# nerficg-project/nerficg

Hardware: AMD Instinct MI355X
Metric: Mrays/s (INGP lego) (higher is better)
Workload: dtype f16 (tables, weights, activations) / f32 (accumulate, march, composite); 1 GPU; ingp_lego: 800x800 image render per rank per step (640000 rays), solid-sphere occupancy r<0.35, random-init hash grid (T=2^19, L=16, F=2) + 64-wide MLPs, seed 0, 100 seeded orbit poses; parallelism=rays x1 (weak)

## Files before the change

### include/nerficg_hip.h

```cpp
#ifndef NERFICG_HIP_H
#define NERFICG_HIP_H

#include <stdint.h>

#ifdef __cplusplus
extern "C" {
#endif

typedef void* nrc_stream_t;

enum {
    NRC_OK = 0,
    NRC_ERR_INVALID = -1,
    NRC_ERR_LAUNCH = -2,
    NRC_ERR_UNSUPPORTED = -3
};

#define NRC_ABI_VERSION 22
int nrc_abi_version(void);
const char* nrc_build_info(void);
const char* nrc_last_error(void);


int nrc_ray_aabb_intersect(const float* rays_o, const float* rays_d, const float* centers, const float* half_sizes,
// ... 269 lines not shown
                             void* view, nrc_stream_t stream);
int nrc_ngp_set_encoder_ypair_view(const void* view);
int nrc_ngp_set_encoder_ypair_levels(int32_t levels);
int nrc_ngp_encode_samples(const float* ts, const int32_t* row_tile, const float* ray_od, int64_t first_row, int64_t n_rows, const float* xyz_min3,
                           const float* xyz_size3, const void* table_f16, int32_t n_levels, int32_t log2_hashmap_size,
                           int32_t base_resolution, float per_level_scale, void* features_f16, const int32_t* arena_tile_off,
                           int32_t arena_rows, nrc_stream_t stream);
int nrc_ngp_mlp_samples(const float* ts, const int32_t* row_tile, const float* ray_od, int64_t first_row, int64_t n_rows, int64_t n_ray_tiles,
                        const void* features_f16, const void* density_weights_f16, const void* color_weights_f16,
                        void* packed_f16, void* ray_sh_workspace, const int32_t* arena_tile_off, int32_t arena_rows, nrc_stream_t stream);
int nrc_ngp_composite_image(const void* packed_f16, const float* ts, const int32_t* ray_cnt, const int32_t* tile_off,
                            int32_t width, int32_t height, int64_t tile_begin, int64_t n_tiles, int32_t cascades,
                            float exp_step_factor, int32_t grid_size, int32_t max_samples, float T_threshold,
                            const float* bg3, float* rgb, float* alpha, float* depth, int64_t row_capacity, int32_t arena_rows,
                            nrc_stream_t stream);
int64_t nrc_ngp_render_frame_ws_bytes(int64_t n_rows, int64_t n_ray_tiles, int32_t max_samples, int64_t row_budget);
int nrc_ngp_render_frame(const float* ts_arena, int32_t* row_tile, const float* ray_od, int64_t n_rows, int64_t n_ray_tiles,
                         const float* xyz_min3, const float* xyz_size3, const void* density_weights_f16, const void* color_weights_f16,
                         const void* table_f16, int32_t n_levels, int32_t log2_hashmap_size, int32_t base_resolution, float per_level_scale,
                         const int32_t* ray_cnt, const int32_t* tile_off, int32_t width, int32_t height, int64_t tile_begin, int32_t cascades,
                         float exp_step_factor, int32_t grid_size, int32_t max_samples, float T_threshold, const float* bg3_host, float* rgb,
                         float* alpha, float* depth, int64_t row_budget, void* workspace, nrc_stream_t stream);

int nrc_ssim_forward(const float* img1, const float* img2, int64_t planes, int32_t H, int32_t W, float C1, float C2, float* ssim_map,
                     float* dm_dmu1, float* dm_dsigma1_sq, float* dm_dsigma12, nrc_stream_t stream);
int nrc_ssim_backward(const float* img1, const float* img2, int64_t planes, int32_t H, int32_t W, const float* dL_dmap,
                      const float* dm_dmu1, const float* dm_dsigma1_sq, const float* dm_dsigma12, float* dL_dimg1,
                      nrc_stream_t stream);
int64_t nrc_photometric_loss_ws_floats(int64_t planes, int32_t H, int32_t W);
int nrc_photometric_loss_forward(const float* image, const float* target, int64_t planes, int32_t H, int32_t W, float C1, float C2,
// ... 229 lines not shown
```

### nerficg_amd/csrc/ngp_net.hip

```cpp
#include "ngp_net.h"
#include "ngp_image_step.h"

namespace {

enum { ENC_GRID = 0, ENC_SH_ID = 1, ENC_FEAT = 2, ENC_DIR_H = 3, ENC_GRID_F2 = 4, ENC_GRID_F4 = 5 };
enum { ACT_NONE = 0, ACT_SIGMOID = 1 };

__device__ __forceinline__ void encode_grid(float px, float py, float pz, int hh, __amdgpu_buffer_rsrc_t table, const GridCfg& g, h8 (&B)[2]) {
#pragma unroll
    for (int s = 0; s < 2; s++) {
#pragma unroll
        for (int q = 0; q < 4; q++) {
            const int l0 = 8 * s + q, l1 = 8 * s + 4 + q;
            const float scale = hh ? g.scale[l1] : g.scale[l0];
            const uint32_t res = hh ? g.res[l1] : g.res[l0];
            const uint32_t size = hh ? g.size[l1] : g.size[l0];
            const uint32_t off = hh ? g.offset[l1] : g.offset[l0];
            const bool hashed = hh ? g.hashed[l1] : g.hashed[l0];
            Corner8 c;
            grid_corners(px, py, pz, scale, res, size, off, hashed, c);
            float f0, f1;
            grid_level_features(table, c, f0, f1);
            B[s][2 * q] = (_Float16)f0;
            B[s][2 * q + 1] = (_Float16)f1;
// ... 226 lines not shown
            px = __fdiv_rn(px, in.sz[0]); py = __fdiv_rn(py, in.sz[1]); pz = __fdiv_rn(pz, in.sz[2]);
        }
        return 1;
    }
}
template <int SRC>
__device__ __forceinline__ void fetch_dir(const QueryIn& in, int64_t i, float& dx, float& dy, float& dz) {
    if constexpr (SRC == SRC_ARRAYS) {
        dx = in.dirs[3 * i]; dy = in.dirs[3 * i + 1]; dz = in.dirs[3 * i + 2];
    } else {
        const float* od = in.ray_od + (int64_t)tile_of(in.row_tile[i >> 6]) * 384 + (i & 63);
        dx = od[192]; dy = od[256]; dz = od[320];
    }
}

template <int SRC>
__global__ void __launch_bounds__(256) k_grid_encode(QueryIn in, int64_t base, int64_t n, const __half2* __restrict__ table, GridCfg g,
                                                         uint4* __restrict__ feat, int narrow_levels, int lvl_range, int lane_shape = 0, int xcd_run = 0,
                                                         BlockView bv = BlockView{}, VertexView vv = VertexView{}, YPairView yv = YPairView{}) {
    int64_t bid = blockIdx.x;
    if constexpr (SRC == SRC_TILED) {
        int64_t first = 0, span = gridDim.x;
        if (xcd_run > 0) {
            const int64_t run = 8 * (int64_t)xcd_run;
            first = bid / run * run;
            span = first + run <= (int64_t)gridDim.x ? run : (int64_t)gridDim.x - first;
        }
        const int64_t g8 = span >> 3, r = bid - first;
        if (r < 8 * g8) bid = first + (r & 7) * g8 + (r >> 3);
    }
    int64_t j = bid * 256 + threadIdx.x;
    bool remapped = false;
    if constexpr (SRC == SRC_TILED) {
        if (in.n_rows_dev) {
// ... 5 lines not shown
            base = r0 * 64;
            n = (r1 - r0) * 64 < n ? (r1 - r0) * 64 : n;
        }
    }
    if constexpr (SRC == SRC_TILED) {
        if (lane_shape != 0) {
            const int lu = (lane_shape >> 4) & 7, lv = lane_shape & 7, ls = 6 - lu - lv;
            const int64_t g1024 = j & ~(int64_t)1023;
            const int w = (int)((j >> 6) & 15), l = (int)(j & 63);
            const int iu = l & ((1 << lu) - 1), iv = (l >> lu) & ((1 << lv) - 1), is = l >> (lu + lv);
            const int gu = w & ((NRC_TILE_W >> lu) - 1), gv = (w >> (NRC_TILE_W_LOG2 - lu)) & ((NRC_TILE_H >> lv) - 1), gs = w >> (6 - lu - lv);
            j = g1024 + ((int64_t)((gs << ls) + is) << 6) + NRC_TILE_W * ((gv << lv) + iv) + (gu << lu) + iu;
            remapped = true;
        }
    }
    if (j >= n || j < 0) return;
    float px, py, pz;
    if (blockIdx.y != 0) in.x01_out = nullptr;
    const int state = remapped ? fetch_pos<SRC, false>(in, base + j, px, py, pz) : fetch_pos<SRC>(in, base + j, px, py, pz);
    if (state < 0) return;
    const bool live = state > 0;
    const __amdgpu_buffer_rsrc_t trs = make_table_rsrc(table, g.total_entries * 4u);
    const __amdgpu_buffer_rsrc_t vrs = make_table_rsrc(bv.ptr, bv.bytes);
    const __amdgpu_buffer_rsrc_t xrs = make_table_rsrc(vv.ptr, vv.bytes);
    const __amdgpu_buffer_rsrc_t yrs = make_table_rsrc(yv.ptr, yv.bytes);
    uint4* out = feat + ((j >> 5) * 4) * 32 + (j & 31);
    const int rot = (int)((j >> 5) & 3);
    const int lvl_lo = lvl_range & 0xff, lvl_hi = (lvl_range >> 8) & 0xff;
    const int grp_begin = gridDim.y == 4 ? (int)blockIdx.y : 0, grp_end = gridDim.y == 4 ? grp_begin + 1 : 4;
#pragma unroll 1
    for (int grp = grp_begin; grp < grp_end; grp++) {
        uint32_t v[4] = {0u, 0u, 0u, 0u};
        if (live) {
#pragma unroll
            for (int q = 0; q < 4; q++) {
                const int level = 4 * grp + q;
                if (level < lvl_lo || level >= lvl_hi) continue;
                Corner8 c;
                float f0, f1;
                if (SRC == SRC_TILED && level < bv.levels) {
                    uint32_t gx, gy, gz;
                    grid_cell(px, py, pz, g.scale[level], gx, gy, gz, c.w);
                    grid_level_features_block(vrs, bv.first[level], gx, gy, gz, g.res[level], c.w, f0, f1);
                } else if (SRC == SRC_TILED && level >= yv.begin && level < yv.begin + yv.levels) {
// ... 5 lines not shown
                    grid_cell(px, py, pz, g.scale[level], gx, gy, gz, c.w);
                    grid_level_features_vertex(xrs, vv.first[level - vv.begin], gx, gy, gz, g.res[level], vv.R[level - vv.begin], c.w, f0, f1);
                } else if (g.hashed[level]) {
                    grid_corners_u<true>(px, py, pz, g.scale[level], g.res[level], g.size[level], g.offset[level], c);
                    grid_level_features_hashed(trs, c, f0, f1);
                } else {
                    grid_corners_u<false>(px, py, pz, g.scale[level], g.res[level], g.size[level], g.offset[level], c);
                    if (level < narrow_levels) grid_level_features_narrow(trs, c, f0, f1);
                    else grid_level_features(trs, c, f0, f1);
                }
                const __half2 h = __floats2half2_rn(f0, f1);
                v[q] = *reinterpret_cast<const uint32_t*>(&h);
                asm volatile("" : "+v"(v[q]));
            }
        }
        out[((grp + rot) & 3) * 32] = make_uint4(v[0], v[1], v[2], v[3]);
    }
}

__global__ void __launch_bounds__(256) k_grid_encode_pairs(QueryIn in, int64_t n, const __half2* __restrict__ table, GridCfg g, uint2* __restrict__ feat,
                                                           int narrow_levels, const int32_t* __restrict__ m_live = nullptr) {
    const int pair = (int)(blockIdx.x & 7u);
    const int64_t j = (int64_t)(blockIdx.x >> 3) * 256 + threadIdx.x;
    if (m_live) n = min(n, ((int64_t)max(*m_live, 0) + 31) / 32 * 32);
    if (j >= n) return;
    float px, py, pz;
    if (pair != 0) in.x01_out = nullptr;
    fetch_pos<SRC_ARRAYS>(in, j, px, py, pz);
    const __amdgpu_buffer_rsrc_t trs = make_table_rsrc(table, g.total_entries * 4u);
    uint32_t* out32 = reinterpret_cast<uint32_t*>(feat);
    const int rot = (int)((j >> 5) & 3);
// ... 70 lines not shown
    const float* od = ray_od + tile * 384 + lane;
    h8 lo, hi;
    sh4_fragments(od[192], od[256], od[320], lo, hi);
    ray_sh[(tile * 2) * 64 + lane] = lo;
    ray_sh[(tile * 2 + 1) * 64 + lane] = hi;
}

__device__ __forceinline__ float fast_sigmoid(float x) { return __builtin_amdgcn_rcpf(1.f + __expf(-x)); }

__device__ __forceinline__ h8 mlp_frag_relu(const f16v& acc, int g) { return acc_to_frag_relu(acc, g); }
__device__ __forceinline__ h8 mlp_frag(const f16v& acc, int g) { return acc_to_frag(acc, g); }
__device__ __forceinline__ f16v mlp_mfma(const h8& a, const h8& b, const f16v& c) { return NRC_MFMA(a, b, c); }
#ifndef NRC_MLP_WAVES
#define NRC_MLP_WAVES 2
#endif
enum { MLP_F_D0 = 0, MLP_F_DO = 4, MLP_F_C0 = 8, MLP_F_C1 = 12, MLP_F_CO = 20, MLP_N_FRAG = 24 };
__device__ __forceinline__ void mlp_stage_weights(h8 (*wlds)[64], const __half* __restrict__ Wd, const __half* __restrict__ Wc) {
    const int lane = threadIdx.x & 63, r = lane & 31, hh = lane >> 5;
    for (int f = threadIdx.x >> 6; f < MLP_N_FRAG; f += 4) {
        h8 v;
        if (f < MLP_F_DO) v = load_w_frag<false>(Wd, 32, 64, (f - MLP_F_D0) >> 1, (f - MLP_F_D0) & 1, r, hh);
        else if (f < MLP_F_C0) v = load_w_head_frag(Wd + 64 * 32, 64, 16, (f - MLP_F_DO) & 1, lane);
        else if (f < MLP_F_C1) {
            const int mt = (f - MLP_F_C0) >> 1, s = (f - MLP_F_C0) & 1;
            v = load_w_frag<false>(Wc, 32, 64, mt, s, r, hh);
        } else if (f < MLP_F_CO) v = load_w_frag<true>(Wc + 64 * 32, 64, 64, (f - MLP_F_C1) >> 2, (f - MLP_F_C1) & 3, r, hh);
        else v = load_w_head_frag(Wc + 64 * 32 + 64 * 64, 64, 16, (f - MLP_F_CO) & 1, lane);
        wlds[f][lane] = v;
    }
}
template <int NT, bool PRE>
__device__ __forceinline__ void mlp_chain_from(const h8 (*wlds)[64], const h8 (&B)[NT][2], const h8 (*X0), const f16v (*P)[2],
                                               _Float16 (&h0)[NT], _Float16 (&rgbh)[NT][3]) {
    const int lane = threadIdx.x & 63;
#define D0(mt, s) wlds[MLP_F_D0 + 2 * (mt) + (s)][lane]
#define DO(s) wlds[MLP_F_DO + (s)][lane]
#define C0(mt, s) wlds[MLP_F_C0 + 2 * (mt) + (s)][lane]
#define C1(mt, s) wlds[MLP_F_C1 + 4 * (mt) + (s)][lane]
#define CO(s) wlds[MLP_F_CO + (s)][lane]
    h8 X[NT][2], H[NT][4];
    f16v acc[NT][2];
    h8 HB[NT][2][2];
    f4v o[NT][2];
#pragma unroll
    for (int u = 0; u < NT; u++) {
        if constexpr (!PRE) X[u][0] = X0[u];
        acc[u][0] = zero16(); acc[u][1] = zero16();
        o[u][0] = f4v{0.f, 0.f, 0.f, 0.f}; o[u][1] = o[u][0];
    }
#pragma unroll
    for (int mt = 0; mt < 2; mt++)
#pragma unroll
        for (int s = 0; s < 2; s++) {
            const h8 w = D0(mt, s);
#pragma unroll
            for (int u = 0; u < NT; u++) acc[u][mt] = mlp_mfma(w, B[u][s], acc[u][mt]);
        }
#pragma unroll
    for (int u = 0; u < NT; u++) {
#pragma unroll
        for (int mt = 0; mt < 2; mt++)
#pragma unroll
            for (int gq = 0; gq < 2; gq++) H[u][2 * mt + gq] = mlp_frag_relu(acc[u][mt], gq);
        head_split(H[u], HB[u]);
    }
#pragma unroll
    for (int s = 0; s < 2; s++) {
        const h8 w = DO(s);
#pragma unroll
        for (int u = 0; u < NT; u++)
#pragma unroll
            for (int nb = 0; nb < 2; nb++) o[u][nb] = NRC_MFMA16(w, HB[u][nb][s], o[u][nb]);
    }
#pragma unroll
    for (int u = 0; u < NT; u++) {
        X[u][1] = head_join(o[u][0], o[u][1]);
        h0[u] = X[u][1][0];
        if constexpr (!PRE) { acc[u][0] = zero16(); acc[u][1] = zero16(); }
    }
#pragma unroll
    for (int mt = 0; mt < 2; mt++)
#pragma unroll
        for (int s = PRE ? 1 : 0; s < 2; s++) {
            const h8 w = C0(mt, s);
#pragma unroll
            for (int u = 0; u < NT; u++) {
                if constexpr (PRE) acc[u][mt] = mlp_mfma(w, X[u][1], P[u][mt]);
                else acc[u][mt] = mlp_mfma(w, X[u][s], acc[u][mt]);
            }
        }
#pragma unroll
    for (int u = 0; u < NT; u++) {
#pragma unroll
        for (int mt = 0; mt < 2; mt++)
#pragma unroll
            for (int gq = 0; gq < 2; gq++) H[u][2 * mt + gq] = mlp_frag_relu(acc[u][mt], gq);
        acc[u][0] = zero16(); acc[u][1] = zero16();
    }
#pragma unroll
    for (int mt = 0; mt < 2; mt++)
#pragma unroll
        for (int s = 0; s < 4; s++) {
            const h8 w = C1(mt, s);
// ... 12 lines not shown
#pragma unroll
    for (int s = 0; s < 2; s++) {
        const h8 w = CO(s);
#pragma unroll
        for (int u = 0; u < NT; u++)
#pragma unroll
            for (int nb = 0; nb < 2; nb++) o[u][nb] = NRC_MFMA16(w, HB[u][nb][s], o[u][nb]);
    }
#pragma unroll
    for (int u = 0; u < NT; u++) {
        float rgb[3];
        head_join_rgb(o[u][0], o[u][1], rgb);
#pragma unroll
        for (int c = 0; c < 3; c++) rgbh[u][c] = (_Float16)fast_sigmoid(rgb[c]);
    }
#undef D0
#undef DO
#undef C1
#undef CO
}
template <int NT>
__device__ __forceinline__ void mlp_chain(const h8 (*wlds)[64], const h8 (&B)[NT][2], const h8 (&X0)[NT], _Float16 (&h0)[NT], _Float16 (&rgbh)[NT][3]) {
    mlp_chain_from<NT, false>(wlds, B, X0, nullptr, h0, rgbh);
}
template <int NT>
__device__ __forceinline__ void mlp_chain(const h8 (*wlds)[64], const h8 (&B)[NT][2], const f16v (&P)[NT][2], _Float16 (&h0)[NT], _Float16 (&rgbh)[NT][3]) {
    mlp_chain_from<NT, true>(wlds, B, nullptr, P, h0, rgbh);
}
template <int NT>
__device__ __forceinline__ void mlp_sh_step(const h8 (*wlds)[64], const h8 (&X0)[NT], f16v (&P)[NT][2]) {
    const int lane = threadIdx.x & 63;
#pragma unroll
    for (int mt = 0; mt < 2; mt++) {
        const h8 w = C0(mt, 0);
// ... 190 lines not shown
    const int incl = nrc_wave_incl_sum_i(v, lane);
    if (lane == 63) wave_tot[wave] = incl;
    __syncthreads();
    int off = incl - v;
    for (int w = 0; w < wave; w++) off += wave_tot[w];
    hist[tid] = off;
    __syncthreads();
    for (int t = t0 + tid; t < t1; t += 1024) order[t0 + atomicAdd(&hist[1023 - min(tile_off[t + 1] - tile_off[t], 1023)], 1)] = t;
    if (tid == 0) {
        chunk_tab[4 * c] = t0; chunk_tab[4 * c + 1] = t1; chunk_tab[4 * c + 2] = tile_off[t0]; chunk_tab[4 * c + 3] = tile_off[t1];
        queue[c] = 0;
    }
}

struct ImageCfg { int width, height, tiles_x; int64_t tile_begin; float esf, dt_min, dt_max, thr, bg_r, bg_g, bg_b; };
__global__ void __launch_bounds__(256, NRC_MLP_WAVES) k_ngp_mlp_composite(const uint4* __restrict__ feat, const h8* __restrict__ ray_sh,
                                                                          const __half* __restrict__ Wd, const __half* __restrict__ Wc,
                                                                          const float* __restrict__ ts, int arena_rows, const int32_t* __restrict__ ray_cnt,
                                                                          const int32_t* __restrict__ tile_off, const int32_t* __restrict__ order,
                                                                          const int32_t* __restrict__ chunk, int32_t* __restrict__ queue, ImageCfg ic,
                                                                          float* __restrict__ rgb, float* __restrict__ alpha_out, float* __restrict__ depth_out) {
    constexpr int NT = 2;
    __shared__ h8 wlds[MLP_N_FRAG][64];
    const int lane = threadIdx.x & 63, r = lane & 31, hh = lane >> 5;
    mlp_stage_weights(wlds, Wd, Wc);
    __syncthreads();
    const int t_first = chunk[0], n_chunk = chunk[1] - chunk[0], row0 = chunk[2];
    auto take = [&]() -> int {
        int q = 0;
        if (lane == 0) q = atomicAdd(queue, 1);
// ... 3 lines not shown
        const int lt = __builtin_amdgcn_readfirstlane(order[t_first + q]);
        const int rb = tile_off[lt], R = tile_off[lt + 1] - rb;
        const int64_t tile = ic.tile_begin + lt;
        const int px = (int)(tile % ic.tiles_x) * NRC_TILE_W + (lane & (NRC_TILE_W - 1)), py = (int)(tile / ic.tiles_x) * NRC_TILE_H + (lane >> NRC_TILE_W_LOG2);
        const bool inside = px < ic.width && py < ic.height;
        const int N = inside ? ray_cnt[(int64_t)lt * 64 + lane] : 0;
        NrcRayAcc acc = nrc_ray_acc(N > 0);
        f16v P[NT][2];
        {
            h8 X0[NT];
#pragma unroll
            for (int u = 0; u < NT; u++) X0[u] = ray_sh[((int64_t)lt * 2 + hh) * 64 + r + 32 * u];
            mlp_sh_step<NT>(wlds, X0, P);
        }
        const float* tcol = ts + (((int64_t)lt * arena_rows) << 6) + lane;
        const uint4* fcol = feat + (int64_t)(rb - row0) * (NT * 128) + r;
        const int rot0 = (2 * (rb - row0)) & 3;
        uint4 nb[NT][2];
        float nt_ = 0.f;
        auto fetch = [&](int k) {
#pragma unroll
            for (int u = 0; u < NT; u++) {
                const uint4* fp = fcol + (int64_t)(2 * k + u) * 128;
                const int rot = (rot0 + 2 * k + u) & 3;
                nb[u][0] = fp[((hh + rot) & 3) * 32];
                nb[u][1] = fp[((2 + hh + rot) & 3) * 32];
            }
            nt_ = tcol[(int64_t)k << 6];
        };
        if (R > 0) fetch(0);
        for (int k = 0; k < R && __any(acc.alive); k++) {
            h8 B[NT][2];
#pragma unroll
            for (int u = 0; u < NT; u++) { B[u][0] = *reinterpret_cast<const h8*>(&nb[u][0]); B[u][1] = *reinterpret_cast<const h8*>(&nb[u][1]); }
            const float t = nt_;
            if (k + 1 < R) fetch(k + 1);
            _Float16 h0[NT], rgbh[NT][3];
            mlp_chain<NT>(wlds, B, P, h0, rgbh);
            uint32_t w01[NT], w23[NT];
#pragma unroll
            for (int u = 0; u < NT; u++) {
                const h2 a = {h0[u], rgbh[u][0]}, b = {rgbh[u][1], rgbh[u][2]};
                w01[u] = *reinterpret_cast<const uint32_t*>(&a);
                w23[u] = *reinterpret_cast<const uint32_t*>(&b);
            }
            const auto s01 = __builtin_amdgcn_permlane32_swap(w01[0], w01[1], false, false);
            const auto s23 = __builtin_amdgcn_permlane32_swap(w23[0], w23[1], false, false);
            const uint32_t p01 = s01[0], p23 = s23[0];
            if (acc.alive && k < N) {
                const float2 f01 = __half22float2(*reinterpret_cast<const __half2*>(&p01));
                const float2 f23 = __half22float2(*reinterpret_cast<const __half2*>(&p23));
                nrc_composite_sample(acc, f01.x, f01.y, f23.x, f23.y, t, ic.esf, ic.dt_min, ic.dt_max, ic.thr, k + 1 >= N);
            }
// ... 162 lines not shown
    const void* view = g_enc_ypair_view;
    g_enc_ypair_view = nullptr;
    return view;
}
static YPairView ypair_view_of(const void* view, const GridCfg& g, int n_levels) {
    YPairView yv;
    ypair_view_cfg(g, n_levels, yv);
    const int want = g_enc_ypair_levels_override >= 0 ? g_enc_ypair_levels_override : NRC_ENC_YPAIR_LEVELS;
    yv.ptr = view;
    if (want < yv.levels) yv.levels = want;
    if (!yv.ptr || yv.levels <= 0) { yv.ptr = nullptr; yv.levels = 0; }
    return yv;
}
template <int SRC>
static void launch_encode(const QueryIn& in, int64_t base, int64_t n, const void* table, const GridCfg& g, uint4* feat, hipStream_t s,
                          const BlockView& bv = BlockView{}, const VertexView& vv = VertexView{}, const YPairView& yv = YPairView{}) {
    int narrow = 0;
    while (narrow < NRC_MAX_LEVELS && !g.hashed[narrow] && g.size[narrow] > 8) narrow++;
    static const int lvl_range = [] {
        const char* e = getenv("NRC_ENC_LEVELS");
        int lo = 0, hi = NRC_MAX_LEVELS;
        if (e && sscanf(e, "%d-%d", &lo, &hi) == 2 && lo >= 0 && hi <= NRC_MAX_LEVELS && lo <= hi) return lo | (hi << 8);
        return NRC_MAX_LEVELS << 8;
    }();
    const int64_t split_below = (int64_t)2 << 20;
    if constexpr (SRC == SRC_ARRAYS) {
        if (n < split_below && base == 0 && lvl_range == (NRC_MAX_LEVELS << 8)) {
            hipLaunchKernelGGL(k_grid_encode_pairs, dim3((unsigned)(8 * nrc_cdiv(n, 256))), dim3(256), 0, s, in, n, (const __half2*)table, g, (uint2*)feat, narrow,
                               in.m_live);
            return;
        }
    }
    const unsigned rows = (SRC == SRC_ARRAYS && n < split_below) ? 4u : 1u;
    const int lane_shape = (3 << 4) | 1;
    const int lanes = (SRC == SRC_TILED && (base & 1023) == 0) ? (g_enc_shape_override ? g_enc_shape_override : lane_shape) : 0;
    hipLaunchKernelGGL(k_grid_encode<SRC>, dim3((unsigned)(lanes ? 4 * nrc_cdiv(n, 1024) : nrc_cdiv(n, 256)), rows), dim3(256), 0, s, in, base, n, (const __half2*)table, g, feat,
                       narrow, lvl_range, lanes, g_enc_xcd_run_override ? g_enc_xcd_run_override : NRC_ENC_XCD_RUN, bv, vv, yv);
}

template <int SRC>
static void launch_mlp(const QueryIn& in, int64_t base, int64_t n, const void* feat, const void* ray_sh, const void* wd, const void* wc,
                       float* sigmas, float* rgbs, void* packed, hipStream_t s) {
    hipLaunchKernelGGL(k_ngp_mlp<SRC>, dim3(pick_blocks(nrc_cdiv(n, 2))), dim3(256), 0, s, in, base, n, (const uint4*)feat, (const h8*)ray_sh,
                       (const __half*)wd, (const __half*)wc, sigmas, rgbs, (__half*)packed);
}

template <int SRC>
static int run_query(const QueryIn& in, int64_t M, int64_t n_ray_tiles, const void* wd, const void* wc, const void* table, const GridCfg& g,
                     float* sigmas, float* rgbs, void* packed, void* workspace, hipStream_t s, const BlockView& bv = BlockView{},
                     const VertexView& vv = VertexView{}, const YPairView& yv = YPairView{}) {
// ... 358 lines not shown
                                    skipped_rows, (int)arena_rows, s);
        base += NRC_QUERY_CHUNK;
    } while (base < M);
    NRC_LAUNCH_CHECK();
    return NRC_OK;
}

#ifndef NRC_FRAME_ROW_BUDGET
#define NRC_FRAME_ROW_BUDGET (int64_t(1) << 21)
#endif
static int64_t frame_budget(int64_t row_budget) { return row_budget > 0 ? row_budget : NRC_FRAME_ROW_BUDGET; }
static int64_t frame_chunks(int64_t n_rows, int64_t budget, int32_t max_samples) {
    return n_rows <= budget ? 1 : nrc_cdiv(n_rows, budget - max_samples);
}
static int64_t round256(int64_t b) { return (b + 255) / 256 * 256; }
int64_t nrc_ngp_render_frame_ws_bytes(int64_t n_rows, int64_t n_ray_tiles, int32_t max_samples, int64_t row_budget) {
    const int64_t budget = frame_budget(row_budget);
    if (n_rows < 0 || n_ray_tiles < 0 || max_samples < 1 || budget < 2 * (int64_t)max_samples) return NRC_ERR_INVALID;
    const int64_t chunks = frame_chunks(n_rows, budget, max_samples);
    const int64_t feat_rows = n_rows < budget ? n_rows : budget;
    return round256((feat_rows > 0 ? feat_rows : 1) * 64 * 64) + round256(n_ray_tiles * 2048) + round256(n_ray_tiles * 4) + round256(chunks * 20);
}

int nrc_ngp_render_frame(const float* ts_arena, int32_t* row_tile, const float* ray_od, int64_t n_rows, int64_t n_ray_tiles, const float* xyz_min3,
                         const float* xyz_size3, const void* density_weights_f16, const void* color_weights_f16, const void* table_f16, int32_t n_levels,
                         int32_t log2_hashmap_size, int32_t base_resolution, float per_level_scale, const int32_t* ray_cnt, const int32_t* tile_off,
                         int32_t width, int32_t height, int64_t tile_begin, int32_t cascades, float exp_step_factor, int32_t grid_size, int32_t max_samples,
                         float T_threshold, const float* bg3_host, float* rgb, float* alpha, float* depth, int64_t row_budget, void* workspace,
                         nrc_stream_t stream) {
    NRC_ENTER();
// ... 2 lines not shown
    const void* yview = take_ypair_view();
    const int64_t budget = frame_budget(row_budget);
    if (n_rows < 0 || n_ray_tiles < 1 || width < 1 || height < 1 || tile_begin < 0 || cascades < 1 || grid_size < 1 || max_samples < 1 ||
        budget < 2 * (int64_t)max_samples || !density_weights_f16 || !color_weights_f16 || !table_f16 || !xyz_min3 || !xyz_size3 || !bg3_host)
        return NRC_ERR_INVALID;
    if (n_levels != 16) return NRC_ERR_UNSUPPORTED;
    if (!ray_od || !ray_cnt || !tile_off || !rgb || !alpha || !depth || !workspace || (n_rows > 0 && (!ts_arena || !row_tile))) return NRC_ERR_INVALID;
    GridCfg g;
    const int rc = make_grid_cfg(n_levels, log2_hashmap_size, base_resolution, per_level_scale, g, nullptr);
    if (rc != NRC_OK) return rc;
    hipStream_t s = (hipStream_t)stream;
    const int64_t chunks = frame_chunks(n_rows, budget, max_samples);
    const int64_t feat_rows = n_rows < budget ? n_rows : budget;
    char* wsp = (char*)workspace;
    uint4* feat = (uint4*)wsp;
    wsp += round256((feat_rows > 0 ? feat_rows : 1) * 64 * 64);
    h8* ray_sh = (h8*)wsp;
    wsp += round256(n_ray_tiles * 2048);
    int32_t* order = (int32_t*)wsp;
    wsp += round256(n_ray_tiles * 4);
    int32_t* chunk_tab = (int32_t*)wsp;
    int32_t* queue = chunk_tab + 4 * chunks;
    QueryIn in = {};
    in.ts = ts_arena; in.row_tile = row_tile; in.ray_od = ray_od; in.tile_off = tile_off; in.arena_rows = max_samples;
    for (int k = 0; k < 3; k++) { in.mn[k] = xyz_min3[k]; in.sz[k] = xyz_size3[k]; }
    ImageCfg ic;
    ic.width = width; ic.height = height; ic.tiles_x = (width + NRC_TILE_W - 1) / NRC_TILE_W; ic.tile_begin = tile_begin;
    ic.esf = exp_step_factor; ic.dt_min = 1.73205080757f / max_samples; ic.dt_max = 1.73205080757f * 2 * (float)cascades / grid_size;
    ic.thr = T_threshold; ic.bg_r = bg3_host[0]; ic.bg_g = bg3_host[1]; ic.bg_b = bg3_host[2];
    int dev = 0, n_cu = 0;
    hipGetDevice(&dev);
    hipDeviceGetAttribute(&n_cu, hipDeviceAttributeMultiprocessorCount, dev);
    const int64_t resident = (int64_t)(n_cu > 0 ? n_cu : 256) * NRC_MLP_WAVES, mlp_blocks = nrc_cdiv(n_ray_tiles, 4) < resident ? nrc_cdiv(n_ray_tiles, 4) : resident;
    const BlockView bv = block_view_of(view, g, n_levels);
    const VertexView vv = vertex_view_of(vview, g, n_levels);
    const YPairView yv = ypair_view_of(yview, g, n_levels);
    NRC_STAGE(s, nullptr);
    hipLaunchKernelGGL(k_ray_sh, dim3((unsigned)nrc_cdiv(n_ray_tiles * 64, 256)), dim3(256), 0, s, ray_od, n_ray_tiles, ray_sh, tile_off, row_tile, n_rows);
    NRC_STAGE(s, "k_ray_sh");
    hipLaunchKernelGGL(k_tile_chunks, dim3((unsigned)chunks), dim3(1024), 0, s, tile_off, n_ray_tiles, chunks > 1 ? budget - max_samples : n_rows + 1,
                       chunk_tab, order, queue);
    NRC_STAGE(s, "k_tile_chunks");
    for (int64_t c = 0; c < chunks; c++) {
        if (n_rows > 0) {
            in.chunk_rows = chunk_tab + 4 * c + 2;
            launch_encode<SRC_TILED>(in, 0, feat_rows * 64, table_f16, g, feat, s, bv, vv, yv);
            NRC_STAGE(s, "k_grid_encode");
        }
        hipLaunchKernelGGL(k_ngp_mlp_composite, dim3((unsigned)mlp_blocks), dim3(256), 0, s, feat, ray_sh, (const __half*)density_weights_f16,
                           (const __half*)color_weights_f16, ts_arena, (int)max_samples, ray_cnt, tile_off, order, chunk_tab + 4 * c, queue + c, ic, rgb, alpha, depth);
        NRC_STAGE(s, "k_ngp_mlp");
    }
    NRC_LAUNCH_CHECK();
    return NRC_OK;
}

}

namespace {

#define LDP 40

__device__ __forceinline__ int img_off(int row, int ch) {
    return 1024 * (row >> 3) + 512 * (ch >> 2) + 64 * (row & 7) + 16 * ((ch & 3) ^ ((row >> 2) & 3));
}
// ... 1312 lines not shown
```

### nerficg_amd/instant_ngp.py

```python
from __future__ import annotations

import ctypes
import math
import warnings
from dataclasses import dataclass, field

import numpy as np
import torch

from . import VolumeRenderingV2 as VolumeRenderingCuda
from . import _lib
from . import tinycudann as tcnn
from .ngp import composite_over_background, query_fused, query_train


def next_multiple(value, multiple: int) -> int:
    return int(((value + multiple - 1) // multiple) * multiple)


@dataclass
class Camera:
    width: int
    height: int
    focal_x: float
# ... 75 lines not shown
        loss, self.last = instant_ngp_loss(outputs['rgb'], rgb, m.encoding_xyz, m.color_mlp_with_encoding, m.n_params_encoding_mlp, m.n_mlp_params,
                                           self.weight_decay_weight)
        return loss

    def psnr(self) -> torch.Tensor:
        return -10.0 * torch.log10(self.last[1])


class InstantNGPRenderer:

    RAY_CHUNK = 1 << 16
    T_THRESHOLD = 1e-4
    COUNT_MAILBOX = True
    POSE_ENCODER_SHAPE = True
    ARENA_IN_PLACE = True
    FRAME_ROW_BUDGET = 0

    def __init__(self, model: InstantNGPModel, MAX_SAMPLES: int = 1024, EXPONENTIAL_STEPS: bool = False, DENSITY_THRESHOLD: float = 0.01) -> None:
        self.model = model
        self.MAX_SAMPLES, self.EXPONENTIAL_STEPS, self.DENSITY_THRESHOLD = MAX_SAMPLES, EXPONENTIAL_STEPS, DENSITY_THRESHOLD
        self.density_threshold = DENSITY_THRESHOLD * MAX_SAMPLES / 3 ** 0.5
        self._fused_ws: dict = {}
        self._box_host = None
        self._scene_box_host = None
        self._zero_center = torch.zeros(1, 3, device=model.center.device)
        self.provisional_march = True
        self.sample_capacity: int | None = None

    @staticmethod
    def _host_copies(cache, tensors):
# ... 250 lines not shown
            return
        m, lib = self.model, _lib.load()
        if not arena:
            _lib.check(lib.nrc_ngp_render_write(nt, _lib.ptr(m.occupancy_bitfield), m.cascades, float(m.SCALE), float(fc['esf']), m.RESOLUTION,
                                                self.MAX_SAMPLES, _lib.ptr(ws['ray_od']), _lib.ptr(ws['ray_t']), _lib.ptr(ws['ray_cnt']),
                                                _lib.ptr(ws['tile_off']), _lib.ptr(ws['ts']), _lib.ptr(ws['row_tile']), _lib.ptr(ws.get('ts_prov')),
                                                int(rows) if fixed else 0, _lib.stream_of(ws['ray_od'])), 'ngp_render_write')
        args = query_args if query_args is not None else self._query_args(fc, ws, nt, fixed, arena)
        args[3] = rows
        if self.POSE_ENCODER_SHAPE:
            lib.nrc_ngp_set_encoder_shape(*fc['enc_shape'])
        self._frame_entry(lib.nrc_ngp_query_samples, args, 'ngp_query_samples', ws['block_view'])

    def _frame_args(self, fc: dict, ws: dict, out: dict, tile_begin: int, nt: int) -> list:
        m, lib, cam, vp, g = self.model, _lib.load(), fc['camera'], ctypes.c_void_p, fc['grid']
        budget = int(self.FRAME_ROW_BUDGET)
        if ws.get('fws_key') != (ws['cap'], budget):
            ws['fws'] = None
            ws['fws'] = torch.empty(int(lib.nrc_ngp_render_frame_ws_bytes(ws['cap'], nt, self.MAX_SAMPLES, budget)), dtype=torch.uint8, device=ws['ray_od'].device)
            ws['fws_key'] = (ws['cap'], budget)
        ws['block_view'] = self._block_view_ptr()
        return [_lib.ptr(ws['ts_prov']), _lib.ptr(ws['row_tile']), _lib.ptr(ws['ray_od']), 0, nt, ctypes.cast(fc['mn'], vp), ctypes.cast(fc['sz'], vp),
                _lib.ptr(m.encoding_xyz._half_params()), _lib.ptr(m.color_mlp_with_encoding._half_params()), _lib.ptr(m.encoding_xyz._table16()),
                g['n_levels'], g['log2_hashmap_size'], g['base_resolution'], float(g['per_level_scale']), _lib.ptr(ws['ray_cnt']), _lib.ptr(ws['tile_off']),
                cam.width, cam.height, int(tile_begin), m.cascades, float(fc['esf']), m.RESOLUTION, self.MAX_SAMPLES, 1e-4, ctypes.cast(fc['bg'], vp),
                _lib.ptr(out['rgb']), _lib.ptr(out['alpha']), _lib.ptr(out['depth']), budget, _lib.ptr(ws['fws']), _lib.stream_of(ws['ray_od'])]

    def _fused_frame(self, fc: dict, ws: dict, out: dict, rows: int, tile_begin: int, nt: int, frame_args: list | None = None) -> None:
        lib = _lib.load()
        args = frame_args if frame_args is not None else self._frame_args(fc, ws, out, tile_begin, nt)
        args[3] = rows
        if self.POSE_ENCODER_SHAPE:
            lib.nrc_ngp_set_encoder_shape(*fc['enc_shape'])
        self._frame_entry(lib.nrc_ngp_render_frame, args, 'ngp_render_frame', ws['block_view'])

    def _fused_composite(self, fc: dict, ws: dict, out: dict, tile_begin: int, nt: int, row_capacity: int = 0, arena: bool = False) -> None:
        m, lib, cam = self.model, _lib.load(), fc['camera']
        _lib.check(lib.nrc_ngp_composite_image(
            _lib.ptr(ws.get('packed')), _lib.ptr(ws.get('ts_prov') if arena else ws.get('ts')), _lib.ptr(ws['ray_cnt']), _lib.ptr(ws['tile_off']), cam.width,
            cam.height, int(tile_begin), nt, m.cascades, float(fc['esf']), m.RESOLUTION, self.MAX_SAMPLES, 1e-4, ctypes.cast(fc['bg'], ctypes.c_void_p),
            _lib.ptr(out['rgb']), _lib.ptr(out['alpha']), _lib.ptr(out['depth']), int(row_capacity), self.MAX_SAMPLES if arena else 0,
            _lib.stream_of(ws['ray_od'])), 'ngp_composite_image')

    @torch.no_grad()
    def render_image_pipelined(self, camera: Camera, c2w: np.ndarray, shards: int = 4, return_stats: bool = False) -> dict[str, torch.Tensor]:
        from .parallel import shard_range
        m = self.model
        dev = m.center.device
# ... 288 lines not shown
```

Baseline: 87.00 Mrays/s.

## Fuse density MLP into grid encoder and pass density output to colour kernel

Adds a density-encoder form of the tiled grid-encode kernel. It stages the density-MLP weights in LDS, regroups the four feature groups across wave halves with permlane32 swaps, runs the density half of the MLP, and writes a single 16-byte density output per sample instead of the 64-byte encoding. The MLP/composite kernel is templated so that, in this mode, it reads that compact output and runs only the colour half. This is meant to cut feature-buffer traffic between the two kernels and remove density work from the composite kernel. In exchange the encoder carries more registers, an LDS footprint, a block barrier and a launch-bounds occupancy target, and out-of-range threads can no longer exit early.

After: 93.80 Mrays/s, median of 6. 1.08x the previous value.

```diff
diff --git a/include/nerficg_hip.h b/include/nerficg_hip.h
--- a/include/nerficg_hip.h
+++ b/include/nerficg_hip.h
@@ -307,6 +307,7 @@
                             float exp_step_factor, int32_t grid_size, int32_t max_samples, float T_threshold,
                             const float* bg3, float* rgb, float* alpha, float* depth, int64_t row_capacity, int32_t arena_rows,
                             nrc_stream_t stream);
+int nrc_ngp_set_frame_density_encoder(int32_t mode);
 int64_t nrc_ngp_render_frame_ws_bytes(int64_t n_rows, int64_t n_ray_tiles, int32_t max_samples, int64_t row_budget);
 int nrc_ngp_render_frame(const float* ts_arena, int32_t* row_tile, const float* ray_od, int64_t n_rows, int64_t n_ray_tiles,
                          const float* xyz_min3, const float* xyz_size3, const void* density_weights_f16, const void* color_weights_f16,
diff --git a/nerficg_amd/csrc/ngp_net.hip b/nerficg_amd/csrc/ngp_net.hip
--- a/nerficg_amd/csrc/ngp_net.hip
+++ b/nerficg_amd/csrc/ngp_net.hip
@@ -264,10 +264,21 @@
     }
 }
 
-template <int SRC>
-__global__ void __launch_bounds__(256) k_grid_encode(QueryIn in, int64_t base, int64_t n, const __half2* __restrict__ table, GridCfg g,
+enum { MLP_F_D0 = 0, MLP_F_DO = 4, MLP_F_C0 = 8, MLP_F_C1 = 12, MLP_F_CO = 20, MLP_N_FRAG = 24 };
+__device__ __forceinline__ void mlp_stage_weights(h8 (*wlds)[64], const __half* __restrict__ Wd, const __half* __restrict__ Wc, int n_frag = MLP_N_FRAG);
+template <int NT>
+__device__ __forceinline__ void mlp_density_half(const h8 (*wlds)[64], const h8 (&B)[NT][2], h8 (&X1)[NT]);
+#ifndef NRC_ENC_DENS_WAVES
+#define NRC_ENC_DENS_WAVES 7
+#endif
+template <int SRC, bool DENS = false>
+__global__ void __launch_bounds__(256, DENS ? NRC_ENC_DENS_WAVES : 0) k_grid_encode(QueryIn in, int64_t base, int64_t n, const __half2* __restrict__ table, GridCfg g,
                                                          uint4* __restrict__ feat, int narrow_levels, int lvl_range, int lane_shape = 0, int xcd_run = 0,
-                                                         BlockView bv = BlockView{}, VertexView vv = VertexView{}, YPairView yv = YPairView{}) {
+                                                         BlockView bv = BlockView{}, VertexView vv = VertexView{}, YPairView yv = YPairView{},
+                                                         const __half* __restrict__ Wd = nullptr) {
+    static_assert(!DENS || SRC == SRC_TILED, "the density-encoder form belongs to the tiled layout");
+    extern __shared__ h8 enc_wlds[][64];
+    if constexpr (DENS) mlp_stage_weights(enc_wlds, Wd, nullptr, MLP_F_DO + 2);
     int64_t bid = blockIdx.x;
     if constexpr (SRC == SRC_TILED) {
         int64_t first = 0, span = gridDim.x;
@@ -303,11 +314,17 @@
             remapped = true;
         }
     }
-    if (j >= n || j < 0) return;
-    float px, py, pz;
+    const bool in_range = j < n && j >= 0;
+    if constexpr (!DENS) {
+        if (!in_range) return;
+    }
+    float px = 0.f, py = 0.f, pz = 0.f;
     if (blockIdx.y != 0) in.x01_out = nullptr;
-    const int state = remapped ? fetch_pos<SRC, false>(in, base + j, px, py, pz) : fetch_pos<SRC>(in, base + j, px, py, pz);
-    if (state < 0) return;
+    int state = -1;
+    if (in_range) state = remapped ? fetch_pos<SRC, false>(in, base + j, px, py, pz) : fetch_pos<SRC>(in, base + j, px, py, pz);
+    if constexpr (!DENS) {
+        if (state < 0) return;
+    }
     const bool live = state > 0;
     const __amdgpu_buffer_rsrc_t trs = make_table_rsrc(table, g.total_entries * 4u);
     const __amdgpu_buffer_rsrc_t vrs = make_table_rsrc(bv.ptr, bv.bytes);
@@ -317,6 +334,7 @@
     const int rot = (int)((j >> 5) & 3);
     const int lvl_lo = lvl_range & 0xff, lvl_hi = (lvl_range >> 8) & 0xff;
     const int grp_begin = gridDim.y == 4 ? (int)blockIdx.y : 0, grp_end = gridDim.y == 4 ? grp_begin + 1 : 4;
+    uint4 F[4] = {};
 #pragma unroll 1
     for (int grp = grp_begin; grp < grp_end; grp++) {
         uint32_t v[4] = {0u, 0u, 0u, 0u};
@@ -352,7 +370,37 @@
                 asm volatile("" : "+v"(v[q]));
             }
         }
-        out[((grp + rot) & 3) * 32] = make_uint4(v[0], v[1], v[2], v[3]);
+        if constexpr (DENS) {
+            F[0] = F[1]; F[1] = F[2]; F[2] = F[3]; F[3] = make_uint4(v[0], v[1], v[2], v[3]);
+        } else {
+            out[((grp + rot) & 3) * 32] = make_uint4(v[0], v[1], v[2], v[3]);
+        }
+    }
+    if constexpr (DENS) {
+        const int lane = threadIdx.x & 63;
+        h8 B[2][1][2];
+#pragma unroll
+        for (int s = 0; s < 2; s++) {
+            const uint4 x = F[2 * s], y = F[2 * s + 1];
+            const auto s0 = __builtin_amdgcn_permlane32_swap(x.x, y.x, false, false);
+            const auto s1 = __builtin_amdgcn_permlane32_swap(x.y, y.y, false, false);
+            const auto s2 = __builtin_amdgcn_permlane32_swap(x.z, y.z, false, false);
+            const auto s3 = __builtin_amdgcn_permlane32_swap(x.w, y.w, false, false);
+            const uint4 a = make_uint4(s0[0], s1[0], s2[0], s3[0]), b = make_uint4(s0[1], s1[1], s2[1], s3[1]);
+            B[0][0][s] = *reinterpret_cast<const h8*>(&a);
+            B[1][0][s] = *reinterpret_cast<const h8*>(&b);
+        }
+        const uint32_t own = (in_range && state >= 0) ? (uint32_t)j : ~0u;
+        const auto slot = __builtin_amdgcn_permlane32_swap(own, own, false, false);
+        __syncthreads();
+#pragma unroll
+        for (int v = 0; v < 2; v++) {
+            h8 X1[1];
+            mlp_density_half<1>(enc_wlds, B[v], X1);
+            const uint32_t sj = slot[v];
+            if (sj != ~0u) feat[(int64_t)(sj >> 5) * 64 + (lane & 32) + (sj & 31u)] = *reinterpret_cast<const uint4*>(&X1[0]);
+            asm volatile("" ::: "memory");
+        }
     }
 }
 
@@ -453,10 +501,9 @@
 #ifndef NRC_MLP_WAVES
 #define NRC_MLP_WAVES 2
 #endif
-enum { MLP_F_D0 = 0, MLP_F_DO = 4, MLP_F_C0 = 8, MLP_F_C1 = 12, MLP_F_CO = 20, MLP_N_FRAG = 24 };
-__device__ __forceinline__ void mlp_stage_weights(h8 (*wlds)[64], const __half* __restrict__ Wd, const __half* __restrict__ Wc) {
+__device__ __forceinline__ void mlp_stage_weights(h8 (*wlds)[64], const __half* __restrict__ Wd, const __half* __restrict__ Wc, int n_frag) {
     const int lane = threadIdx.x & 63, r = lane & 31, hh = lane >> 5;
-    for (int f = threadIdx.x >> 6; f < MLP_N_FRAG; f += 4) {
+    for (int f = threadIdx.x >> 6; f < n_frag; f += 4) {
         h8 v;
         if (f < MLP_F_DO) v = load_w_frag<false>(Wd, 32, 64, (f - MLP_F_D0) >> 1, (f - MLP_F_D0) & 1, r, hh);
         else if (f < MLP_F_C0) v = load_w_head_frag(Wd + 64 * 32, 64, 16, (f - MLP_F_DO) & 1, lane);
@@ -468,22 +515,20 @@
         wlds[f][lane] = v;
     }
 }
-template <int NT, bool PRE>
-__device__ __forceinline__ void mlp_chain_from(const h8 (*wlds)[64], const h8 (&B)[NT][2], const h8 (*X0), const f16v (*P)[2],
-                                               _Float16 (&h0)[NT], _Float16 (&rgbh)[NT][3]) {
-    const int lane = threadIdx.x & 63;
 #define D0(mt, s) wlds[MLP_F_D0 + 2 * (mt) + (s)][lane]
 #define DO(s) wlds[MLP_F_DO + (s)][lane]
 #define C0(mt, s) wlds[MLP_F_C0 + 2 * (mt) + (s)][lane]
 #define C1(mt, s) wlds[MLP_F_C1 + 4 * (mt) + (s)][lane]
 #define CO(s) wlds[MLP_F_CO + (s)][lane]
-    h8 X[NT][2], H[NT][4];
+template <int NT>
+__device__ __forceinline__ void mlp_density_half(const h8 (*wlds)[64], const h8 (&B)[NT][2], h8 (&X1)[NT]) {
+    const int lane = threadIdx.x & 63;
+    h8 H[NT][4];
     f16v acc[NT][2];
     h8 HB[NT][2][2];
     f4v o[NT][2];
 #pragma unroll
     for (int u = 0; u < NT; u++) {
-        if constexpr (!PRE) X[u][0] = X0[u];
         acc[u][0] = zero16(); acc[u][1] = zero16();
         o[u][0] = f4v{0.f, 0.f, 0.f, 0.f}; o[u][1] = o[u][0];
     }
@@ -512,9 +557,19 @@
             for (int nb = 0; nb < 2; nb++) o[u][nb] = NRC_MFMA16(w, HB[u][nb][s], o[u][nb]);
     }
 #pragma unroll
+    for (int u = 0; u < NT; u++) X1[u] = head_join(o[u][0], o[u][1]);
+}
+template <int NT, bool PRE>
+__device__ __forceinline__ void mlp_colour_half(const h8 (*wlds)[64], const h8 (&X1)[NT], const h8 (*X0), const f16v (*P)[2],
+                                                _Float16 (&h0)[NT], _Float16 (&rgbh)[NT][3]) {
+    const int lane = threadIdx.x & 63;
+    h8 H[NT][4];
+    f16v acc[NT][2];
+    h8 HB[NT][2][2];
+    f4v o[NT][2];
+#pragma unroll
     for (int u = 0; u < NT; u++) {
-        X[u][1] = head_join(o[u][0], o[u][1]);
-        h0[u] = X[u][1][0];
+        h0[u] = X1[u][0];
         if constexpr (!PRE) { acc[u][0] = zero16(); acc[u][1] = zero16(); }
     }
 #pragma unroll
@@ -524,8 +579,8 @@
             const h8 w = C0(mt, s);
 #pragma unroll
             for (int u = 0; u < NT; u++) {
-                if constexpr (PRE) acc[u][mt] = mlp_mfma(w, X[u][1], P[u][mt]);
-                else acc[u][mt] = mlp_mfma(w, X[u][s], acc[u][mt]);
+                if constexpr (PRE) acc[u][mt] = mlp_mfma(w, X1[u], P[u][mt]);
+                else acc[u][mt] = mlp_mfma(w, s == 0 ? X0[u] : X1[u], acc[u][mt]);
             }
         }
 #pragma unroll
@@ -568,10 +623,17 @@
 #pragma unroll
         for (int c = 0; c < 3; c++) rgbh[u][c] = (_Float16)fast_sigmoid(rgb[c]);
     }
+}
 #undef D0
 #undef DO
 #undef C1
 #undef CO
+template <int NT, bool PRE>
+__device__ __forceinline__ void mlp_chain_from(const h8 (*wlds)[64], const h8 (&B)[NT][2], const h8 (*X0), const f16v (*P)[2],
+                                               _Float16 (&h0)[NT], _Float16 (&rgbh)[NT][3]) {
+    h8 X1[NT];
+    mlp_density_half<NT>(wlds, B, X1);
+    mlp_colour_half<NT, PRE>(wlds, X1, X0, P, h0, rgbh);
 }
 template <int NT>
 __device__ __forceinline__ void mlp_chain(const h8 (*wlds)[64], const h8 (&B)[NT][2], const h8 (&X0)[NT], _Float16 (&h0)[NT], _Float16 (&rgbh)[NT][3]) {
@@ -792,6 +854,7 @@
 }
 
 struct ImageCfg { int width, height, tiles_x; int64_t tile_begin; float esf, dt_min, dt_max, thr, bg_r, bg_g, bg_b; };
+template <bool DENS>
 __global__ void __launch_bounds__(256, NRC_MLP_WAVES) k_ngp_mlp_composite(const uint4* __restrict__ feat, const h8* __restrict__ ray_sh,
                                                                           const __half* __restrict__ Wd, const __half* __restrict__ Wc,
                                                                           const float* __restrict__ ts, int arena_rows, const int32_t* __restrict__ ray_cnt,
@@ -825,29 +888,43 @@
             mlp_sh_step<NT>(wlds, X0, P);
         }
         const float* tcol = ts + (((int64_t)lt * arena_rows) << 6) + lane;
-        const uint4* fcol = feat + (int64_t)(rb - row0) * (NT * 128) + r;
+        const uint4* fcol = DENS ? feat + (int64_t)(rb - row0) * (NT * 64) + lane : feat + (int64_t)(rb - row0) * (NT * 128) + r;
         const int rot0 = (2 * (rb - row0)) & 3;
-        uint4 nb[NT][2];
+        uint4 nb[NT][DENS ? 1 : 2];
         float nt_ = 0.f;
         auto fetch = [&](int k) {
 #pragma unroll
             for (int u = 0; u < NT; u++) {
-                const uint4* fp = fcol + (int64_t)(2 * k + u) * 128;
-                const int rot = (rot0 + 2 * k + u) & 3;
-                nb[u][0] = fp[((hh + rot) & 3) * 32];
-                nb[u][1] = fp[((2 + hh + rot) & 3) * 32];
+                if constexpr (DENS) {
+                    nb[u][0] = fcol[(int64_t)(2 * k + u) * 64];
+                } else {
+                    const uint4* fp = fcol + (int64_t)(2 * k + u) * 128;
+                    const int rot = (rot0 + 2 * k + u) & 3;
+                    nb[u][0] = fp[((hh + rot) & 3) * 32];
+                    nb[u][1] = fp[((2 + hh + rot) & 3) * 32];
+                }
             }
             nt_ = tcol[(int64_t)k << 6];
         };
         if (R > 0) fetch(0);
         for (int k = 0; k < R && __any(acc.alive); k++) {
-            h8 B[NT][2];
-#pragma unroll
-            for (int u = 0; u < NT; u++) { B[u][0] = *reinterpret_cast<const h8*>(&nb[u][0]); B[u][1] = *reinterpret_cast<const h8*>(&nb[u][1]); }
+            h8 B[NT][DENS ? 1 : 2];
+#pragma unroll
+            for (int u = 0; u < NT; u++) {
+                B[u][0] = *reinterpret_cast<const h8*>(&nb[u][0]);
+                if constexpr (!DENS) B[u][1] = *reinterpret_cast<const h8*>(&nb[u][1]);
+            }
             const float t = nt_;
             if (k + 1 < R) fetch(k + 1);
             _Float16 h0[NT], rgbh[NT][3];
-            mlp_chain<NT>(wlds, B, P, h0, rgbh);
+            if constexpr (DENS) {
+                h8 X1[NT];
+#pragma unroll
+                for (int u = 0; u < NT; u++) X1[u] = B[u][0];
+                mlp_colour_half<NT, true>(wlds, X1, nullptr, P, h0, rgbh);
+            } else {
+                mlp_chain<NT>(wlds, B, P, h0, rgbh);
+            }
             uint32_t w01[NT], w23[NT];
 #pragma unroll
             for (int u = 0; u < NT; u++) {
@@ -1040,7 +1117,8 @@
 }
 template <int SRC>
 static void launch_encode(const QueryIn& in, int64_t base, int64_t n, const void* table, const GridCfg& g, uint4* feat, hipStream_t s,
-                          const BlockView& bv = BlockView{}, const VertexView& vv = VertexView{}, const YPairView& yv = YPairView{}) {
+                          const BlockView& bv = BlockView{}, const VertexView& vv = VertexView{}, const YPairView& yv = YPairView{},
+                          const void* density_weights = nullptr) {
     int narrow = 0;
     while (narrow < NRC_MAX_LEVELS && !g.hashed[narrow] && g.size[narrow] > 8) narrow++;
     static const int lvl_range = [] {
@@ -1060,6 +1138,14 @@
     const unsigned rows = (SRC == SRC_ARRAYS && n < split_below) ? 4u : 1u;
     const int lane_shape = (3 << 4) | 1;
     const int lanes = (SRC == SRC_TILED && (base & 1023) == 0) ? (g_enc_shape_override ? g_enc_shape_override : lane_shape) : 0;
+    if constexpr (SRC == SRC_TILED) {
+        if (density_weights) {
+            hipLaunchKernelGGL((k_grid_encode<SRC_TILED, true>), dim3((unsigned)(lanes ? 4 * nrc_cdiv(n, 1024) : nrc_cdiv(n, 256))), dim3(256),
+                               (MLP_F_DO + 2) * 64 * sizeof(h8), s, in, base, n, (const __half2*)table, g, feat, narrow, lvl_range, lanes,
+                               g_enc_xcd_run_override ? g_enc_xcd_run_override : NRC_ENC_XCD_RUN, bv, vv, yv, (const __half*)density_weights);
+            return;
+        }
+    }
     hipLaunchKernelGGL(k_grid_encode<SRC>, dim3((unsigned)(lanes ? 4 * nrc_cdiv(n, 1024) : nrc_cdiv(n, 256)), rows), dim3(256), 0, s, in, base, n, (const __half2*)table, g, feat,
                        narrow, lvl_range, lanes, g_enc_xcd_run_override ? g_enc_xcd_run_override : NRC_ENC_XCD_RUN, bv, vv, yv);
 }
@@ -1448,6 +1534,19 @@
     return n_rows <= budget ? 1 : nrc_cdiv(n_rows, budget - max_samples);
 }
 static int64_t round256(int64_t b) { return (b + 255) / 256 * 256; }
+#ifndef NRC_FRAME_DENSITY_ENCODER
+#define NRC_FRAME_DENSITY_ENCODER 1
+#endif
+static thread_local int g_frame_density_override = -1;
+static bool frame_density_pair(int64_t feat_rows) {
+    const int want = g_frame_density_override >= 0 ? g_frame_density_override : NRC_FRAME_DENSITY_ENCODER;
+    return want != 0 && feat_rows <= (int64_t(1) << 24);
+}
+int nrc_ngp_set_frame_density_encoder(int32_t mode) {
+    if (mode < -1 || mode > 1) return NRC_ERR_INVALID;
+    g_frame_density_override = mode;
+    return NRC_OK;
+}
 int64_t nrc_ngp_render_frame_ws_bytes(int64_t n_rows, int64_t n_ray_tiles, int32_t max_samples, int64_t row_budget) {
     const int64_t budget = frame_budget(row_budget);
     if (n_rows < 0 || n_ray_tiles < 0 || max_samples < 1 || budget < 2 * (int64_t)max_samples) return NRC_ERR_INVALID;
@@ -1480,6 +1579,7 @@
     const int64_t feat_rows = n_rows < budget ? n_rows : budget;
     char* wsp = (char*)workspace;
     uint4* feat = (uint4*)wsp;
+    const bool dens = frame_density_pair(feat_rows);
     wsp += round256((feat_rows > 0 ? feat_rows : 1) * 64 * 64);
     h8* ray_sh = (h8*)wsp;
     wsp += round256(n_ray_tiles * 2048);
@@ -1510,11 +1610,15 @@
     for (int64_t c = 0; c < chunks; c++) {
         if (n_rows > 0) {
             in.chunk_rows = chunk_tab + 4 * c + 2;
-            launch_encode<SRC_TILED>(in, 0, feat_rows * 64, table_f16, g, feat, s, bv, vv, yv);
+            launch_encode<SRC_TILED>(in, 0, feat_rows * 64, table_f16, g, feat, s, bv, vv, yv, dens ? density_weights_f16 : nullptr);
             NRC_STAGE(s, "k_grid_encode");
         }
-        hipLaunchKernelGGL(k_ngp_mlp_composite, dim3((unsigned)mlp_blocks), dim3(256), 0, s, feat, ray_sh, (const __half*)density_weights_f16,
-                           (const __half*)color_weights_f16, ts_arena, (int)max_samples, ray_cnt, tile_off, order, chunk_tab + 4 * c, queue + c, ic, rgb, alpha, depth);
+        if (dens)
+            hipLaunchKernelGGL(k_ngp_mlp_composite<true>, dim3((unsigned)mlp_blocks), dim3(256), 0, s, feat, ray_sh, (const __half*)density_weights_f16,
+                               (const __half*)color_weights_f16, ts_arena, (int)max_samples, ray_cnt, tile_off, order, chunk_tab + 4 * c, queue + c, ic, rgb, alpha, depth);
+        else
+            hipLaunchKernelGGL(k_ngp_mlp_composite<false>, dim3((unsigned)mlp_blocks), dim3(256), 0, s, feat, ray_sh, (const __half*)density_weights_f16,
+                               (const __half*)color_weights_f16, ts_arena, (int)max_samples, ray_cnt, tile_off, order, chunk_tab + 4 * c, queue + c, ic, rgb, alpha, depth);
         NRC_STAGE(s, "k_ngp_mlp");
     }
     NRC_LAUNCH_CHECK();
diff --git a/nerficg_amd/instant_ngp.py b/nerficg_amd/instant_ngp.py
--- a/nerficg_amd/instant_ngp.py
+++ b/nerficg_amd/instant_ngp.py
@@ -113,6 +113,7 @@
     COUNT_MAILBOX = True
     POSE_ENCODER_SHAPE = True
     ARENA_IN_PLACE = True
+    FRAME_DENSITY_ENCODER = -1
     FRAME_ROW_BUDGET = 0
 
     def __init__(self, model: InstantNGPModel, MAX_SAMPLES: int = 1024, EXPONENTIAL_STEPS: bool = False, DENSITY_THRESHOLD: float = 0.01) -> None:
@@ -393,11 +394,12 @@
 
     def _frame_args(self, fc: dict, ws: dict, out: dict, tile_begin: int, nt: int) -> list:
         m, lib, cam, vp, g = self.model, _lib.load(), fc['camera'], ctypes.c_void_p, fc['grid']
-        budget = int(self.FRAME_ROW_BUDGET)
-        if ws.get('fws_key') != (ws['cap'], budget):
+        budget, pair = int(self.FRAME_ROW_BUDGET), int(self.FRAME_DENSITY_ENCODER)
+        _lib.check(lib.nrc_ngp_set_frame_density_encoder(pair), 'ngp_set_frame_density_encoder')
+        if ws.get('fws_key') != (ws['cap'], budget, pair):
             ws['fws'] = None
             ws['fws'] = torch.empty(int(lib.nrc_ngp_render_frame_ws_bytes(ws['cap'], nt, self.MAX_SAMPLES, budget)), dtype=torch.uint8, device=ws['ray_od'].device)
-            ws['fws_key'] = (ws['cap'], budget)
+            ws['fws_key'] = (ws['cap'], budget, pair)
         ws['block_view'] = self._block_view_ptr()
         return [_lib.ptr(ws['ts_prov']), _lib.ptr(ws['row_tile']), _lib.ptr(ws['ray_od']), 0, nt, ctypes.cast(fc['mn'], vp), ctypes.cast(fc['sz'], vp),
                 _lib.ptr(m.encoding_xyz._half_params()), _lib.ptr(m.color_mlp_with_encoding._half_params()), _lib.ptr(m.encoding_xyz._table16()),
@@ -411,6 +413,7 @@
         args[3] = rows
         if self.POSE_ENCODER_SHAPE:
             lib.nrc_ngp_set_encoder_shape(*fc['enc_shape'])
+        lib.nrc_ngp_set_frame_density_encoder(ws['fws_key'][2])
         self._frame_entry(lib.nrc_ngp_render_frame, args, 'ngp_render_frame', ws['block_view'])
 
     def _fused_composite(self, fc: dict, ws: dict, out: dict, tile_begin: int, nt: int, row_capacity: int = 0, arena: bool = False) -> None:
```
